# microsoft/crescent-credentials

Hardware: AMD Instinct MI355X
Metric: Groth16 proofs/sec (rs256-sd-shaped circuit, BN254), G1 MSM scalar-adds/sec reported alongside (higher is better)
Workload: dtype u32 limbs (BN254 Fq/Fr, 254-bit modular integers)

## Files before the change

crescent-credentials_amd/csrc/msm.hip:

```cpp
#include "msm.hpp"
#include "g2pair.hpp"

#include <chrono>
#include <cstring>
#include <type_traits>

namespace cg {

static constexpr int SCALAR_BITS = 255;

int msm_default_window(uint64_t n, bool precomputed) {
    double best = 1e300;
    int best_c = 4;
    for (int c = 4; c <= 22; ++c) {
        int W = (SCALAR_BITS + c - 1) / c;
        if ((double)W * (double)n >= 2147483648.0) continue;
        double buckets = (double)(1u << (c - 1)) * (precomputed ? 1 : W);
        if (buckets > (double)(1u << 24)) continue;
        double cost = (double)n * W * 12.0 + buckets * 2.0 * 16.0;
        if (cost < best) { best = cost; best_c = c; }
    }
    return best_c;
}

// ... 188 lines not shown
    if constexpr (I < N) {
        f(std::integral_constant<int, I>{});
        static_for<I + 1, N>(f);
    }
}
template <int C, class Fn>
__device__ __forceinline__ void for_each_digit_c(const uint32_t (&s)[8], Fn f) {
    constexpr int W = (SCALAR_BITS + C - 1) / C;
    constexpr uint32_t mask = (1u << C) - 1u, half = 1u << (C - 1);
    int hl = -1;
    uint32_t top = 0;
#pragma unroll
    for (int i = 0; i < 8; ++i) {
        hl = s[i] ? i : hl;
        top = s[i] ? s[i] : top;
    }
    if (hl < 0) return;
    const int topbit = hl * 32 + 31 - __clz((int)top);
    uint32_t carry = 0;
    bool live = true;
    static_for<0, W>([&](auto jc) __attribute__((always_inline)) {
        constexpr int j = decltype(jc)::value;
        constexpr int bit = C * j, lo = bit >> 5, sh = bit & 31;
        if (!live) return;
        if (bit > topbit && carry == 0) { live = false; return; }
        uint32_t w = 0;
        if constexpr (lo < 8) {
            if constexpr (sh == 0) w = s[lo];
            else if constexpr (lo + 1 < 8) w = __builtin_amdgcn_alignbit(s[lo + 1], s[lo], sh);
            else w = s[lo] >> sh;
        }
        const uint32_t raw = (w & mask) + carry;
        int32_t d;
        if (raw > half) { d = (int32_t)raw - (int32_t)(1u << C); carry = 1; }
        else { d = (int32_t)raw; carry = 0; }
        f(j, d);
    });
}

static constexpr int PART_MAX_BITS = 12;
static constexpr uint32_t PART_TILE = 4096;
static constexpr uint32_t PART_THREADS = 1024;
static constexpr uint32_t PART_CHUNK = 8192;
static constexpr uint32_t PART_PAD = 16;
enum { PLAN_N = 0, PLAN_L = 1, PLAN_T = 2, PLAN_NONZERO = 3, PLAN_CHUNKS = 4, PLAN_DONE = 5, PLAN_WORDS = 8 };

struct PartShape {
    uint32_t n;
    int c, W;
    int precomputed;
    uint32_t row_stride;
    int bits1, bits2;
    int staged;
};

__device__ __forceinline__ Fr load_scalar_or_zero(const Fr* __restrict__ scalars, uint32_t i, bool ok) {
    uint4 a = make_uint4(0u, 0u, 0u, 0u), b = a;
    if (ok) {
        const uint4* p = reinterpret_cast<const uint4*>(scalars + i);
        a = p[0];
        b = p[1];
    }
    Fr r;
    r.l[0] = a.x; r.l[1] = a.y; r.l[2] = a.z; r.l[3] = a.w;
    r.l[4] = b.x; r.l[5] = b.y; r.l[6] = b.z; r.l[7] = b.w;
    return r;
}

template <int C, class Fn>
__device__ __forceinline__ void for_each_entry(const PartShape& sh, const Fr& s, uint32_t i, Fn f) {
    const uint32_t nb = 1u << (sh.c - 1);
    auto emit = [&](int j, int32_t d) {
        if (d == 0) return;
        const uint32_t mag = (uint32_t)(d < 0 ? -d : d);
        const uint32_t sign = d < 0 ? 0x80000000u : 0u;
        if (sh.precomputed) f(mag - 1u, ((uint32_t)j * sh.row_stride + i) | sign);
        else f((uint32_t)j * nb + (mag - 1u), i | sign);
    };
    if constexpr (C > 0) for_each_digit_c<C>(s.l, emit);
    else for_each_digit(s.l, sh.c, sh.W, emit);
}

struct PlanArgs {
    uint32_t* start1;
    uint32_t* chunk0;
    uint32_t target_threads, min_L;
    int two_level;
};
__device__ __forceinline__ uint32_t block_exclusive_scan(uint32_t* sc, uint32_t n);
__device__ __forceinline__ void part_plan_block(int bits1, const PlanArgs& pa, const uint32_t* hist1, uint32_t* plan, uint32_t* lds);

template <int C>
__global__ void __launch_bounds__(PART_THREADS) k_part_count(PartShape sh, const Fr* __restrict__ scalars, const uint8_t* __restrict__ valid,
                                                    uint32_t* __restrict__ blk_hist, uint32_t* hist1, uint32_t* plan, PlanArgs pa) {
    extern __shared__ uint32_t lds[];
    const uint32_t B1 = 1u << sh.bits1;
    for (uint32_t k = threadIdx.x; k < B1; k += blockDim.x) lds[k] = 0;
    __syncthreads();
    const uint32_t base = blockIdx.x * PART_TILE;
    uint32_t nonzero = 0;
    constexpr int PER = PART_TILE / PART_THREADS;
    Fr sc[PER];
    bool ok[PER];
#pragma unroll
    for (int u = 0; u < PER; ++u) {
        const uint32_t i = base + u * PART_THREADS + threadIdx.x;
        ok[u] = i < sh.n && valid[i] != 0;
        sc[u] = load_scalar_or_zero(scalars, i, ok[u]);
    }
    static_for<0, PER>([&](auto uc) {
        constexpr int u = decltype(uc)::value;
        if (!ok[u]) return;
        bool any = false;
        for_each_entry<C>(sh, sc[u], base + u * PART_THREADS + threadIdx.x, [&](uint32_t key, uint32_t) {
            atomicAdd(&lds[key >> sh.bits2], 1u);
            any = true;
        });
        nonzero += any;
    });
    __shared__ uint32_t nz_block;
    if (threadIdx.x == 0) nz_block = 0;
    for (int off = 32; off > 0; off >>= 1) nonzero += __shfl_down((int)nonzero, off, 64);
    __syncthreads();
    if ((threadIdx.x & 63) == 0 && nonzero) atomicAdd(&nz_block, nonzero);
    __syncthreads();
    if (threadIdx.x == 0 && nz_block) atomicAdd(&plan[PLAN_NONZERO], nz_block);
    uint32_t* row = blk_hist + (size_t)blockIdx.x * B1;
    for (uint32_t k = threadIdx.x; k < B1; k += blockDim.x) {
        const uint32_t v = lds[k];
        row[k] = v;
        if (v) atomicAdd(&hist1[(size_t)k * PART_PAD], v);
    }
    __shared__ uint32_t is_last;
    __builtin_amdgcn_s_waitcnt(0x0F70);
    __builtin_amdgcn_fence(__ATOMIC_RELEASE, "workgroup");
    __syncthreads();
    if (threadIdx.x == 0)
        is_last = __hip_atomic_fetch_add(&plan[PLAN_DONE], 1u, __ATOMIC_RELAXED, __HIP_MEMORY_SCOPE_AGENT) == gridDim.x - 1u;
    __syncthreads();
    if (!is_last) return;
    part_plan_block(sh.bits1, pa, hist1, plan, lds);
}

__device__ __forceinline__ uint32_t block_exclusive_scan(uint32_t* sc, uint32_t n) {
    __shared__ uint32_t wave_tot[16];
    __shared__ uint32_t grand;
    const uint32_t per = (n + blockDim.x - 1) / blockDim.x;
    const uint32_t lo = threadIdx.x * per, hi = lo + per < n ? lo + per : n;
    uint32_t sum = 0;
    for (uint32_t k = lo; k < hi; ++k) sum += sc[k];
    uint32_t incl = sum;
    for (int off = 1; off < 64; off <<= 1) {
        uint32_t v = (uint32_t)__shfl_up((int)incl, off, 64);
        if ((threadIdx.x & 63) >= (uint32_t)off) incl += v;
    }
    if ((threadIdx.x & 63) == 63) wave_tot[threadIdx.x >> 6] = incl;
    __syncthreads();
    if (threadIdx.x == 0) {
        uint32_t run = 0;
        for (uint32_t w = 0; w < (blockDim.x + 63) / 64; ++w) { uint32_t t = wave_tot[w]; wave_tot[w] = run; run += t; }
        grand = run;
    }
    __syncthreads();
    uint32_t run = wave_tot[threadIdx.x >> 6] + incl - sum;
    for (uint32_t k = lo; k < hi; ++k) { uint32_t t = sc[k]; sc[k] = run; run += t; }
    __syncthreads();
    return grand;
}

__device__ __forceinline__ void part_plan_block(int bits1, const PlanArgs& pa, const uint32_t* hist1, uint32_t* plan, uint32_t* lds) {
    const uint32_t B1 = 1u << bits1;
    auto hist = [&](uint32_t k) { return __hip_atomic_load(&hist1[(size_t)k * PART_PAD], __ATOMIC_RELAXED, __HIP_MEMORY_SCOPE_AGENT); };
    __syncthreads();
    for (uint32_t k = threadIdx.x; k < B1; k += blockDim.x) lds[k] = hist(k);
    __syncthreads();
    const uint32_t N = block_exclusive_scan(lds, B1);
    for (uint32_t k = threadIdx.x; k < B1; k += blockDim.x) pa.start1[k] = lds[k];
    if (threadIdx.x == 0) {
        pa.start1[B1] = N;
        uint32_t L = (uint32_t)(((uint64_t)N + pa.target_threads - 1) / pa.target_threads);
        if (L < pa.min_L) L = pa.min_L;
        plan[PLAN_N] = N;
        plan[PLAN_L] = L;
        plan[PLAN_T] = N ? (N + L - 1) / L : 0;
    }
    if (!pa.two_level) return;
    __syncthreads();
    for (uint32_t k = threadIdx.x; k < B1; k += blockDim.x) lds[k] = (hist(k) + PART_CHUNK - 1) / PART_CHUNK;
    __syncthreads();
    const uint32_t chunks = block_exclusive_scan(lds, B1);
    for (uint32_t k = threadIdx.x; k < B1; k += blockDim.x) pa.chunk0[k] = lds[k];
    if (threadIdx.x == 0) { pa.chunk0[B1] = chunks; plan[PLAN_CHUNKS] = chunks; }
}

__global__ void k_replan(uint32_t* __restrict__ plan, const uint32_t* __restrict__ src_plan, uint32_t target_segments, uint32_t min_L) {
    for (int k = 0; k < PLAN_WORDS; ++k) plan[k] = src_plan[k];
    const uint32_t N = plan[PLAN_N];
    uint32_t L = (uint32_t)(((uint64_t)N + target_segments - 1) / target_segments);
    if (L < min_L) L = min_L;
    plan[PLAN_L] = L;
    plan[PLAN_T] = N ? (N + L - 1) / L : 0;
}

template <int C>
__global__ void __launch_bounds__(PART_THREADS) k_part_place(PartShape sh, const Fr* __restrict__ scalars, const uint8_t* __restrict__ valid,
                                                    const uint32_t* __restrict__ blk_hist, const uint32_t* __restrict__ start1,
                                                    uint32_t* __restrict__ cur1, uint64_t* __restrict__ out) {
    extern __shared__ uint32_t lds[];
    const uint32_t B1 = 1u << sh.bits1;
    const uint32_t* row = blk_hist + (size_t)blockIdx.x * B1;
    for (uint32_t k = threadIdx.x; k < B1; k += blockDim.x) {
        const uint32_t cnt = row[k];
        lds[k] = cnt ? start1[k] + atomicAdd(&cur1[(size_t)k * PART_PAD], cnt) : 0u;
    }
    const uint32_t base = blockIdx.x * PART_TILE;
    constexpr int PER = PART_TILE / PART_THREADS;
    Fr sc[PER];
    bool ok[PER];
#pragma unroll
    for (int u = 0; u < PER; ++u) {
        const uint32_t i = base + u * PART_THREADS + threadIdx.x;
        ok[u] = i < sh.n && valid[i] != 0;
        sc[u] = load_scalar_or_zero(scalars, i, ok[u]);
    }
    __syncthreads();
    static_for<0, PER>([&](auto uc) {
        constexpr int u = decltype(uc)::value;
        if (!ok[u]) return;
        for_each_entry<C>(sh, sc[u], base + u * PART_THREADS + threadIdx.x, [&](uint32_t key, uint32_t val) {
            const uint32_t pos = atomicAdd(&lds[key >> sh.bits2], 1u);
            out[pos] = ((uint64_t)key << 32) | val;
        });
    });
}

static constexpr uint32_t STAGE_SUB = 1024;
static constexpr int STAGE_MIN_C = 18;
template <int C>
__global__ void __launch_bounds__(PART_THREADS) k_part_place_staged(PartShape sh, const Fr* __restrict__ scalars, const uint8_t* __restrict__ valid,
                                                           const uint32_t* __restrict__ blk_hist, const uint32_t* __restrict__ start1,
                                                           uint32_t* __restrict__ cur1, uint64_t* __restrict__ out) {
    constexpr int W = (SCALAR_BITS + C - 1) / C;
    extern __shared__ __attribute__((aligned(16))) uint32_t lds[];
    const uint32_t B1 = 1u << sh.bits1;
    uint32_t* gbase = lds;
    uint32_t* cnt = lds + B1;
    uint32_t* off = lds + 2 * B1;
    uint64_t* stage = reinterpret_cast<uint64_t*>(lds + 3 * B1 + (B1 & 1u));
    const uint32_t* row = blk_hist + (size_t)blockIdx.x * B1;
    for (uint32_t k = threadIdx.x; k < B1; k += blockDim.x) {
        const uint32_t c = row[k];
        gbase[k] = c ? start1[k] + atomicAdd(&cur1[(size_t)k * PART_PAD], c) : 0u;
    }
    const uint32_t base = blockIdx.x * PART_TILE;
    for (uint32_t sub = 0; sub < PART_TILE / STAGE_SUB; ++sub) {
        const uint32_t i = base + sub * STAGE_SUB + threadIdx.x;
        for (uint32_t k = threadIdx.x; k < B1; k += blockDim.x) cnt[k] = 0;
        __syncthreads();
        uint64_t e[W];
#pragma unroll
        for (int u = 0; u < W; ++u) e[u] = ~0ull;
        if (i < sh.n && valid[i] != 0) {
            const Fr sc = scalars[i];
            for_each_digit_c<C>(sc.l, [&](int j, int32_t d) {
                if (d == 0) return;
                const uint32_t key = (uint32_t)(d < 0 ? -d : d) - 1u;
                const uint32_t val = ((uint32_t)j * sh.row_stride + i) | (d < 0 ? 0x80000000u : 0u);
                e[j] = ((uint64_t)key << 32) | val;
                atomicAdd(&cnt[key >> sh.bits2], 1u);
            });
        }
        __syncthreads();
        for (uint32_t k = threadIdx.x; k < B1; k += blockDim.x) off[k] = cnt[k];
        __syncthreads();
        const uint32_t total = block_exclusive_scan(off, B1);
        for (uint32_t k = threadIdx.x; k < B1; k += blockDim.x) cnt[k] = off[k];
        __syncthreads();
#pragma unroll
        for (int u = 0; u < W; ++u)
            if (e[u] != ~0ull) stage[atomicAdd(&cnt[(uint32_t)(e[u] >> 32) >> sh.bits2], 1u)] = e[u];
        __syncthreads();
        for (uint32_t k = threadIdx.x; k < total; k += blockDim.x) {
            const uint64_t v = stage[k];
            const uint32_t b = (uint32_t)(v >> 32) >> sh.bits2;
            out[gbase[b] + (k - off[b])] = v;
        }
// ... 796 lines not shown
    for (int k = 0; k < PLAN_WORDS; ++k) h_plan.p[k] = 0;
    h_result.alloc((size_t)wins * (red_rbits + red_cbits1) * ACC);
    if (!ev_t[0])
        for (auto& e : ev_t) CG_HIP(hipEventCreate(&e));
}

template <class F>
void MsmEngine<F>::device_bytes(uint64_t& entries, uint64_t& pieces, uint64_t& other) const {
    entries += own_mem.entry_bytes();
    pieces += own_mem.piece_bytes();
    other += blk_hist.bytes() + counters.bytes() + starts.bytes() + bucket_sums.bytes() + rows_buf.bytes() + cols_buf.bytes() +
             rowp_buf.bytes() + colp_buf.bytes();
}

static float elapsed_ms(hipEvent_t a, hipEvent_t b) {
    float ms = 0;
    if (hipEventElapsedTime(&ms, a, b) != hipSuccess) return 0.f;
    return ms;
}
template <class F> float MsmEngine<F>::ms_total() const { return elapsed_ms(ev_t[0], ev_t[5]); }
template <class F> float MsmEngine<F>::ms_sort() const { return n_scalars ? elapsed_ms(ev_t[1], ev_t[2]) : 0.f; }
template <class F> float MsmEngine<F>::ms_accum() const { return n_scalars ? elapsed_ms(ev_t[3], ev_t[4]) : 0.f; }

template <class F>
MsmEngine<F>::~MsmEngine() {
    for (auto& e : ev_t) if (e) (void)hipEventDestroy(e);
}

template <class F>
void MsmEngine<F>::digits(const Fr* scalars_dev, uint64_t n, hipStream_t st) {
    if (n > bases->n) n = bases->n;
    n_scalars = n;
    adopted = nullptr;
    for (int k = 0; k < PLAN_WORDS; ++k) h_plan.p[k] = 0;
    CG_HIP(hipEventRecord(ev_t[0], st));
    if (!n) {
        if (!counters_clean) fill_zero(counters.p, (counters.bytes() + 15) & ~(size_t)15, st);
        counters_clean = zero_at_end;
        return;
    }
    const uint32_t B1 = 1u << bits1;
    uint32_t* plan = counters.p;
    uint32_t* hist1 = plan + PLAN_WORDS;
    uint32_t* cur1 = hist1 + (size_t)B1 * PART_PAD;
    uint32_t* hist2 = cur1 + (size_t)B1 * PART_PAD;
    uint32_t* cur2 = hist2 + (bits2 ? ((size_t)1 << (bits1 + bits2)) : 0);
    uint32_t* start1 = starts.p;
    uint32_t* chunk0 = starts.p + B1 + 1;
    PartShape sh;
    sh.n = (uint32_t)n; sh.c = bases->c; sh.W = bases->W; sh.precomputed = bases->precomputed ? 1 : 0;
    sh.row_stride = (uint32_t)bases->n;
    sh.bits1 = bits1; sh.bits2 = bits2;
    sh.staged = latency_mode ? 1 : 0;
    const uint32_t tiles = ceil_div(n, PART_TILE);
    CG_HIP(hipEventRecord(ev_t[1], st));
    if (!counters_clean) fill_zero(counters.p, (counters.bytes() + 15) & ~(size_t)15, st);
    counters_clean = false;
    PlanArgs pa;
    pa.start1 = start1; pa.chunk0 = chunk0; pa.target_threads = acc_target_segments<F29T>(latency_mode); pa.min_L = min_L;
    pa.two_level = bits2 ? 1 : 0;
    launch_part_level1(true, sh, tiles, (size_t)B1 * 4, st, scalars_dev, bases->valid.p, blk_hist.p, hist1, plan, nullptr, nullptr, nullptr, pa);
    CG_KERNEL_CHECK();
    launch_part_level1(false, sh, tiles, (size_t)B1 * 4, st, scalars_dev, bases->valid.p, blk_hist.p, nullptr, nullptr, start1, cur1, mem().ent_a.p, pa);
    CG_KERNEL_CHECK();
    if (bits2) {
        const uint32_t B2 = 1u << bits2;
        k_part_count2<<<max_chunks, 256, (size_t)B2 * 4, st>>>(bits1, bits2, mem().ent_a.p, chunk0, start1, hist2);
        CG_KERNEL_CHECK();
        k_part_place2<<<max_chunks, 256, (size_t)B2 * 16 + (size_t)PART_CHUNK * 8, st>>>(bits1, bits2, mem().ent_a.p, chunk0, start1, hist2, cur2, mem().ent_b.p);
        CG_KERNEL_CHECK();
    }
    CG_HIP(hipEventRecord(ev_t[2], st));
}

template <class F>
void MsmEngine<F>::adopt(const uint64_t* grouped_entries, const uint32_t* plan_dev, uint64_t n, hipStream_t st) {
    if (n > bases->n) n = bases->n;
    n_scalars = n;
    for (int k = 0; k < PLAN_WORDS; ++k) h_plan.p[k] = 0;
    CG_HIP(hipEventRecord(ev_t[0], st));
    CG_HIP(hipEventRecord(ev_t[1], st));
    k_replan<<<1, 1, 0, st>>>(counters.p, plan_dev, acc_target_segments<F29T>(latency_mode), min_L);
    counters_clean = false;
    CG_KERNEL_CHECK();
    CG_HIP(hipEventRecord(ev_t[2], st));
    adopted = n ? grouped_entries : nullptr;
}

static bool red_force_tree() {
    static const bool v = CG_TUNE_ENV("RED_TREE") != nullptr;
    return v;
}

template <class F>
void MsmEngine<F>::accumulate(hipStream_t st, bool defer_reduction) {
    reduction_pending = false;
    if (!buckets_clean) fill_zero(bucket_sums.p, bucket_sums.bytes(), st);
    buckets_clean = false;
    if (n_scalars) {
        const uint32_t* plan = counters.p;
        const uint64_t* grouped = adopted ? adopted : this->grouped();
        CG_HIP(hipEventRecord(ev_t[3], st));
        static const bool knock_accum = CG_TUNE_ENV("KNOCK_ACCUM") != nullptr, knock_combine = CG_TUNE_ENV("KNOCK_COMBINE") != nullptr;
        if (!knock_accum)
            launch_accum_affine<F29T>(grouped, plan, max_segments, bases->table.p, bucket_sums.p, mem().part_keys_a.p, mem().part_pts_a.p, latency_mode, st);
        CG_KERNEL_CHECK();
// ... 285 lines not shown
```

crescent-credentials_amd/csrc/msm.hpp:

```cpp
#pragma once
#include "common.hpp"
#include "curve29.hpp"
#include "ntt.hpp"

#include <functional>

namespace cg {

template <class F>
struct MsmBases {
    typedef typename To29<F>::type F29T;
    static constexpr int AFF = Words29<F29T>::AFF;
    uint64_t n = 0;
    int c = 0;
    int W = 0;
    bool precomputed = true;
    DevBuf<uint32_t> table;
    DevBuf<uint8_t> valid;
    void build(const Affine<F>* bases_dev, uint64_t n, int c, bool precompute, hipStream_t st);
    void build_from_row0(const uint32_t* row0_dev, const uint8_t* valid_dev, uint64_t n, int c, hipStream_t st);
    int rebuild(int c_new, hipStream_t st);
    void alloc_rows(uint64_t n, int c, bool precompute);
    void expand_rows(hipStream_t st);
};

int msm_default_window(uint64_t n, bool precomputed);
int msm_best_window(uint64_t n_bases, double nz_small, double nz_full);

struct MsmScratch {
    DevBuf<uint64_t> ent_a, ent_b;
    DevBuf<uint32_t> part_keys_a, part_keys_b;
    DevBuf<uint32_t> part_pts_a, part_pts_b;
    uint64_t entry_bytes() const { return ent_a.bytes() + ent_b.bytes(); }
    uint64_t piece_bytes() const { return part_keys_a.bytes() + part_keys_b.bytes() + part_pts_a.bytes() + part_pts_b.bytes(); }
    void reserve(size_t n_ent_a, size_t n_ent_b, size_t keys_a, size_t pts_a, size_t keys_b, size_t pts_b) {
        if (ent_a.n < n_ent_a) ent_a.alloc(n_ent_a);
        if (ent_b.n < n_ent_b) ent_b.alloc(n_ent_b);
        if (part_keys_a.n < keys_a) part_keys_a.alloc(keys_a);
        if (part_pts_a.n < pts_a) part_pts_a.alloc(pts_a);
        if (part_keys_b.n < keys_b) part_keys_b.alloc(keys_b);
        if (part_pts_b.n < pts_b) part_pts_b.alloc(pts_b);
    }
};

template <class F>
struct MsmEngine {
    typedef typename To29<F>::type F29T;
    static constexpr int ACC = Words29<F29T>::ACC;
    const MsmBases<F>* bases = nullptr;
    uint64_t cap_entries = 0;
    uint32_t nbuckets_total = 0;
    MsmScratch own_mem;
    MsmScratch* shared_mem = nullptr;
    MsmScratch& mem() { return shared_mem ? *shared_mem : own_mem; }
    const MsmScratch& mem() const { return shared_mem ? *shared_mem : own_mem; }
    int bits1 = 0, bits2 = 0;
    DevBuf<uint32_t> blk_hist;
    DevBuf<uint32_t> counters;
    DevBuf<uint32_t> starts;
    uint32_t max_chunks = 0;
    uint32_t min_L = 16;
    uint32_t max_segments = 0;
    DevBuf<uint32_t> bucket_sums;
    DevBuf<uint32_t> rows_buf, cols_buf;
    DevBuf<uint32_t> rowp_buf, colp_buf;
    int red_rbits = 0, red_cbits1 = 0;
    PinnedBuf<uint32_t> h_plan;
    PinnedBuf<uint32_t> h_result;
    uint64_t n_scalars = 0;
    bool zero_at_end = false;
    bool counters_clean = false, buckets_clean = false;
    bool latency_mode = false;
    uint32_t n_entries() const { return h_plan.p ? h_plan.p[0] : 0; }
    uint32_t n_nonzero() const { return h_plan.p ? h_plan.p[3] : 0; }
    void enqueue_reduction(hipStream_t st);
    bool reduction_pending = false;
    hipEvent_t ev_t[6] = {nullptr, nullptr, nullptr, nullptr, nullptr, nullptr};
    float ms_total() const;
    float ms_sort() const;
    float ms_accum() const;

    void init(const MsmBases<F>* b, hipStream_t zero_stream = nullptr);
    ~MsmEngine();
    void device_bytes(uint64_t& entries, uint64_t& pieces, uint64_t& other) const;
    void digits(const Fr* scalars_dev, uint64_t n, hipStream_t st);
    template <class G>
    bool can_adopt(const MsmEngine<G>& src) const {
        return bases->precomputed && src.bases->precomputed && bases->n == src.bases->n && bases->c == src.bases->c &&
               bits1 == src.bits1 && bits2 == src.bits2;
    }
    void adopt(const uint64_t* grouped_entries, const uint32_t* plan_dev, uint64_t n, hipStream_t st);
    const uint64_t* grouped() const { return bits2 ? mem().ent_b.p : mem().ent_a.p; }
    const uint64_t* adopted = nullptr;
    void accumulate(hipStream_t st, bool defer_reduction = false);
    XYZZ<F> value() const;
};

void enqueue_reduction_batch(MsmEngine<Fq>* const* engines, int n, hipStream_t st);

void ec_inverse_dft(const uint32_t* row0_in, const uint8_t* valid_in, uint64_t n_in, int logn, const Fr& scale_base,
                    const Fr& scale_mult, uint32_t* row0_out, uint8_t* valid_out, hipStream_t st);
void ec_transform_h_bases(const uint32_t* row0_in, const uint8_t* valid_in, uint64_t n_in, int logn, uint32_t* row0_out,
                          uint8_t* valid_out, hipStream_t st);
void ec_fold_c_into_l(const uint32_t* h_row0, const uint8_t* h_valid, uint64_t n_h, int logn, const Fr& vanishing_inv,
                      const cg_csr& c_matrix, uint64_t num_constraints, uint64_t num_inputs, uint64_t M,
                      const uint32_t* l_row0, const uint8_t* l_valid, uint32_t* row0_out, uint8_t* valid_out, hipStream_t st);
void ec_fold_ct_into_l(const uint32_t* h_row0, const uint8_t* h_valid, uint64_t n_h, int logn, const Fr& vanishing_inv,
                       const HostCsc& c_transposed, uint64_t num_constraints, uint64_t num_inputs, uint64_t M,
                       const uint32_t* l_row0, const uint8_t* l_valid, uint32_t* row0_out, uint8_t* valid_out, hipStream_t st);
void sum_xyzz_by_key(const uint32_t* keys, const uint32_t* pts, uint64_t count, uint32_t* sums, hipStream_t st);
void build_hl_bases_folded(MsmBases<Fq>& out_h, MsmBases<Fq>& out_l, const Affine<Fq>* h_bases_dev, uint64_t n_h, int logn,
                           const Affine<Fq>* l_bases_dev, uint64_t num_inputs, uint64_t M, const cg_csr& c_matrix,
                           uint64_t num_constraints, const Fr& vanishing_inv, uint64_t h_first, uint64_t h_stride, uint64_t h_count,
                           int c_h, uint64_t l_first, uint64_t l_count, int c_l, hipStream_t st, float* ms_fold = nullptr,
                           float* ms_tables = nullptr);

void build_h_bases_folded(MsmBases<Fq>& out_h, const uint32_t* h_row0, const uint8_t* h_valid, uint64_t n_h, int logn, uint64_t h_first,
                          uint64_t h_stride, uint64_t h_count, int c_h, hipStream_t st, float* ms_fold, float* ms_tables);
void build_l_bases_folded(MsmBases<Fq>& out_l, const uint32_t* h_row0, const uint8_t* h_valid, uint64_t n_h, int logn,
                          const uint32_t* l_row0, const uint8_t* l_valid, uint64_t num_inputs, uint64_t M, const HostCsc& c_transposed,
                          uint64_t num_constraints, const Fr& vanishing_inv, uint64_t l_first, uint64_t l_count,
                          const std::function<int()>& pick_c_l, hipStream_t st, float* ms_fold, float* ms_tables);

template <class F>
void import_bases(const uint8_t* host_bytes, uint32_t coord_form, uint64_t n, Affine<F>* out_dev, hipStream_t st);
// ... 8 lines not shown
```

crescent-credentials_amd/csrc/prover.hip:

```cpp
#include <atomic>
#include <condition_variable>
#include <shared_mutex>
#include <memory>
#include <mutex>
#include <chrono>
#include <cstdlib>
#include <exception>
#include <functional>
#include <thread>

#include "msm.hpp"
#include "ntt.hpp"
#include "scalar_form.hpp"
#include "wmap29.hpp"

namespace cg {

const char* csr_view_problem(const cg_csr& m);

std::string& last_error() {
    static thread_local std::string e;
    return e;
}
int fail(int code, const char* fmt, ...) {
// ... 357 lines not shown

template <class F>
static void load_query(MsmBases<F>& bases, const uint8_t* bytes, uint32_t form, uint64_t first, uint64_t count, int window_bits,
                       bool precompute, hipStream_t st, float* ms_copy, float* ms_tables) {
    constexpr size_t PT = sizeof(Affine<F>);
    auto t0 = std::chrono::steady_clock::now();
    DevBuf<Affine<F>> tmp(count ? count : 1);
    import_bases<F>(bytes + first * PT, form, count, tmp.p, st);
    if (ms_copy) *ms_copy += ms_since(t0);
    t0 = std::chrono::steady_clock::now();
    int c = window_bits > 0 ? window_bits : msm_default_window(count ? count : 1, precompute);
    bases.build(tmp.p, count, c, precompute, st);
    CG_HIP(hipStreamSynchronize(st));
    if (ms_tables) *ms_tables += ms_since(t0);
}

struct SlotRecipe { size_t dev_bytes = 0, host_bytes = 0; };
static std::unique_ptr<ProofSlot> make_slot(cg_ctx* c, const KeyTables& tables, hipStream_t zs, SlotRecipe& rec, bool lone = false,
                                            const std::vector<hipStream_t>& borrow = {}) {
    CG_HIP(hipSetDevice(c->device));
    std::unique_ptr<ProofSlot> sl(new ProofSlot());
    sl->lone = lone;
    AllocMeter meter;
    if (rec.dev_bytes) {
        sl->arena.reset(new SlotArena());
        DevBuf<uint8_t> whole(rec.dev_bytes);
        sl->arena->dev = whole.p; sl->arena->dev_size = rec.dev_bytes;
        whole.p = nullptr; whole.n = 0;
        if (rec.host_bytes) {
            CG_HIP(hipHostMalloc((void**)&sl->arena->host, rec.host_bytes, hipHostMallocDefault));
            sl->arena->host_size = rec.host_bytes;
        }
    }
    ArenaScope carve(sl->arena.get(), rec.dev_bytes ? nullptr : &meter);
    bool serial = !c->latency && !lone;
    if (const char* e = CG_TUNE_ENV("SERIAL_STREAMS")) serial = e[0] == '1' && !lone;
    const bool chain_prio = CG_TUNE_ENV("CHAIN_PRIORITY") && CG_TUNE_ENV("CHAIN_PRIORITY")[0] == '1';
    int prio_lo = 0, prio_hi = 0;
    (void)hipDeviceGetStreamPriorityRange(&prio_lo, &prio_hi);
    for (int i = 0; i < 5; ++i) {
        if (serial && i) sl->st[i] = sl->st[0];
        else if ((size_t)i < borrow.size()) { sl->st[i] = borrow[i]; sl->st_borrowed[i] = true; }
        else if (chain_prio && i == 0) CG_HIP(hipStreamCreateWithPriority(&sl->st[i], hipStreamNonBlocking, prio_hi));
        else CG_HIP(hipStreamCreateWithFlags(&sl->st[i], hipStreamNonBlocking));
    }
    CG_HIP(hipEventCreateWithFlags(&sl->ev_w, hipEventDisableTiming));
    CG_HIP(hipEventCreateWithFlags(&sl->ev_b1, hipEventDisableTiming));
    CG_HIP(hipEventCreateWithFlags(&sl->ev_done, hipEventDisableTiming));
    for (auto& e : sl->ev_fin) CG_HIP(hipEventCreateWithFlags(&e, hipEventDisableTiming));
    sl->one_stream = serial;
    for (auto& e : sl->ev_t) CG_HIP(hipEventCreate(&e));
    const bool latency = c->latency || lone;
    const bool zero_at_end = serial && !(CG_TUNE_ENV("NO_ZERO_AT_END") && CG_TUNE_ENV("NO_ZERO_AT_END")[0] == '1');
    each_query([&](int, auto& e, const auto& t) {
        e.latency_mode = latency;
        if (serial) e.shared_mem = &sl->scratch;
        e.zero_at_end = zero_at_end;
        e.init(&t, zs);
    }, *sl, tables);
    if (c->external_q) {
        sl->h_canon.alloc(c->rh.hi - c->rh.lo ? c->rh.hi - c->rh.lo : 1);
        sl->wm.h_bad_input.alloc(1);
    } else {
        sl->h_canon.alloc(c->D);
        sl->wm.alloc(c->M, c->D, std::max(c->A.sell_scratch, std::max(c->B.sell_scratch, c->C.sell_scratch)));
    }
    if (!rec.dev_bytes) { rec.dev_bytes = meter.dev_bytes + 4096; rec.host_bytes = meter.host_bytes + 4096; }
    return sl;
}

static void add_lone_slot(cg_ctx* c, std::vector<std::unique_ptr<ProofSlot>>& slots, const KeyTables& tables, hipStream_t zs) {
    if (c->n_lone <= 0) return;
    try {
        SlotRecipe own;
        size_t next = slots.size();
        for (int k = 0; k < c->n_lone; ++k) {
            std::vector<hipStream_t> borrow;
            while (borrow.size() < 5 && next > 2 && !slots[next - 1]->lone) borrow.push_back(slots[--next]->st[0]);
            slots.push_back(make_slot(c, tables, zs, own, true, borrow));
        }
    } catch (const HipError& e) {
        if (e.code != CG_ERR_OUT_OF_MEMORY) throw;
        (void)hipGetLastError();
    }
}

struct JoinAll {
    std::vector<std::thread> th;
    ~JoinAll() { for (auto& t : th) if (t.joinable()) t.join(); }
};

struct WorkerCancelled {};
static void staged_worker(cg_ctx* c) {
    const auto t0 = std::chrono::steady_clock::now();
    int status = 0;
    std::string err;
    bool done = false, from_proof = false;
    float ms_fold = 0.f, ms_tables = 0.f, ms_slots = 0.f, ms_wait = 0.f;
    try {
        CG_HIP(hipSetDevice(c->device));
        KeyTables tables;
        const KeyTables& row0 = c->tables;
        std::vector<std::unique_ptr<ProofSlot>> slots;
        int64_t table_bytes = 0;
        auto stop = [&] { if (c->cancel.load()) throw WorkerCancelled(); };
        const uint64_t D = c->D, M = c->M, l = c->l;
        const int wb = c->window_opt;
        TuneStats ts;
// ... 1111 lines not shown
```

crescent-credentials_amd/csrc/wmap29.hip:

```cpp
#include "wmap29.hpp"
#include "satcheck.hpp"

namespace cg {

static constexpr int TS29_SMALL = 10, TS29_BIG = 11;
static int strided_max_stages(int tile_log) { return tile_log == TS29_BIG ? 10 : 6; }
static int ntt_passes(int logn, int tile_log) {
    if (logn <= tile_log) return 1;
    const int smax = strided_max_stages(tile_log);
    return 1 + (logn - tile_log + smax - 1) / smax;
}
static int ntt_tile_log(int logn) {
    static const int forced = [] {
        const char* e = CG_TUNE_ENV("NTT_TILE");
        return (e && (atoi(e) == TS29_SMALL || atoi(e) == TS29_BIG)) ? atoi(e) : 0;
    }();
    if (forced) return (forced == TS29_BIG && logn > TS29_SMALL) ? TS29_BIG : TS29_SMALL;
    return (logn >= 20 && ntt_passes(logn, TS29_BIG) < ntt_passes(logn, TS29_SMALL)) ? TS29_BIG : TS29_SMALL;
}

__device__ __forceinline__ Fr29 load_packed29(const uint32_t* __restrict__ base, uint64_t idx) {
    const uint4* p = reinterpret_cast<const uint4*>(base + idx * 8);
    uint4 a = p[0], b = p[1];
    uint32_t w[8] = {a.x, a.y, a.z, a.w, b.x, b.y, b.z, b.w};
// ... 58 lines not shown
        k_to_packed29<<<ceil_div(n, 256), 256, 0, st>>>(d.icoset_br.p, icoset.p, n, 1, logn);
    }
    CG_KERNEL_CHECK();
    Fr29 v = from_mont256<Fr29P>(d.vanishing_inv);
    pack29(v, vinv);
    Fr vp = from_mont(d.vanishing_inv);
    memcpy(vinv_plain, vp.l, 32);
}

void Wm29Strided::build(const NttDomain& big, int logs_, int rank, hipStream_t st) {
    logs = logs_;
    d = big.n >> logs;
    NttDomain small;
    small.build(big.logn - logs, false, st);
    sub.build(small, st);
    const Fr s = mul(fr_from_u64(5), fr_pow_u64(fr_root_of_unity(big.logn), (uint64_t)rank));
    DevBuf<Fr> t(big.n);
    fr_pow_table(t.p, s, inv(fr_from_u64(big.n)), big.n, false, big.logn, st);
    fold.alloc(big.n * 8);
    k_to_packed29<<<ceil_div(big.n, 256), 256, 0, st>>>(t.p, fold.p, big.n, 0, 0);
    CG_KERNEL_CHECK();
    CG_HIP(hipStreamSynchronize(st));
}

__global__ void __launch_bounds__(256) k_fold29(const uint32_t* __restrict__ a, const uint32_t* __restrict__ T, uint32_t* __restrict__ out,
                                                uint32_t d, int logd, uint32_t terms) {
    const uint32_t i = blockIdx.x * blockDim.x + threadIdx.x;
    if (i >= d) return;
    Fr29 acc = Fr29::zero();
    for (uint32_t t = 0; t < terms; ++t) {
        const uint64_t e = (uint64_t)i + (uint64_t)t * d;
        acc = add(acc, mul(load_packed29(a, e), load_packed29(T, e)));
        if ((t & 3u) == 3u) acc = normalize(acc);
        if ((t & 63u) == 63u) acc = weak_reduce(acc);
    }
    store_packed29(out, brev(i, logd), weak_reduce(normalize(acc)));
}

void Csr29::build(const DevCsr& m, hipStream_t st) {
    dict.alloc(m.dict.n * 8);
    k_to_packed29<<<ceil_div(m.dict.n, 256), 256, 0, st>>>(m.dict.p, dict.p, m.dict.n, 0, 0);
    CG_KERNEL_CHECK();
}

__device__ __forceinline__ bool fr_lt_modulus(const Fr& x) {
    bool lt = false, decided = false;
#pragma unroll
    for (int k = 7; k >= 0; --k) {
        if (!decided && x.l[k] != FrP::N[k]) { lt = x.l[k] < FrP::N[k]; decided = true; }
    }
    return lt;
}

__global__ void __launch_bounds__(256) k_w_to29(const Fr* __restrict__ w, uint32_t* __restrict__ out, uint64_t n,
                                                uint32_t* __restrict__ bad_input, uint32_t* __restrict__ va, uint64_t m, uint64_t l, int logn) {
    uint64_t i = (uint64_t)blockIdx.x * blockDim.x + threadIdx.x;
    if (i >= n) return;
    Fr x = w[i];
    if (!fr_lt_modulus(x)) *bad_input = 1u;
    const Fr29 v = mul(unpack29<Fr29P>(x.l), Fr29::from_limbs(Fr29P::R2));
    store_packed29(out, i, v);
    if (i < l) store_packed29(va, brev((uint32_t)(m + i), logn), v);
}


__global__ void __launch_bounds__(256) k_sell29(const uint32_t* __restrict__ slice_ptr, const uint32_t* __restrict__ col,
                                                const uint32_t* __restrict__ cidx, const uint32_t* __restrict__ dst,
                                                const uint32_t* __restrict__ dict, const uint32_t* __restrict__ src,
                                                uint32_t* __restrict__ out, uint32_t* __restrict__ scratch, uint32_t n_pieces, int logn) {
    const uint32_t p = blockIdx.x * blockDim.x + threadIdx.x;
    if (p >= n_pieces) return;
    const uint32_t s = p >> 6, lane = p & 63u;
    const uint32_t base = slice_ptr[s], len = (slice_ptr[s + 1] - base) >> 6;
    Fr29 acc = Fr29::zero();
    uint32_t cnt = 0;
#if !defined(CG_SELL_BATCH)
#define CG_SELL_BATCH 0
#endif
#if CG_SELL_BATCH == 0
    for (uint32_t t = 0; t < len; ++t) {
        const uint32_t ci = cidx[base + t * 64 + lane];
        if (ci == SELL_PAD) continue;
        Fr29 v = load_packed29(src, col[base + t * 64 + lane]);
        if (ci != 0) v = mul(v, load_packed29(dict, ci));
        acc = add(acc, v);
        if ((++cnt & 3u) == 0) acc = normalize(acc);
    }
#else
    constexpr uint32_t BS = CG_SELL_BATCH;
    uint32_t ci[SELL_PIECE], cl[SELL_PIECE];
#pragma unroll
    for (uint32_t t = 0; t < SELL_PIECE; ++t) {
        const bool in = t < len;
        ci[t] = in ? cidx[base + t * 64 + lane] : SELL_PAD;
        cl[t] = in ? col[base + t * 64 + lane] : 0u;
    }
#pragma unroll
    for (uint32_t h = 0; h < SELL_PIECE; h += BS) {
        if (h >= len) break;
        uint4 rv[BS][2], rd[BS][2];
#pragma unroll
        for (uint32_t u = 0; u < BS; ++u) {
            const uint32_t t = h + u;
            if (ci[t] == SELL_PAD) continue;
            const uint4* pv = reinterpret_cast<const uint4*>(src + (uint64_t)cl[t] * 8);
            rv[u][0] = pv[0]; rv[u][1] = pv[1];
            if (ci[t] != 0) {
                const uint4* pd = reinterpret_cast<const uint4*>(dict + (uint64_t)ci[t] * 8);
                rd[u][0] = pd[0]; rd[u][1] = pd[1];
            }
        }
#pragma unroll
        for (uint32_t u = 0; u < BS; ++u) {
            const uint32_t t = h + u;
            if (ci[t] == SELL_PAD) continue;
// ... 210 lines not shown
    if (threadIdx.x == 0) { rec[0] = 0ull; rec[1] = ~0ull; }
}
__global__ void __launch_bounds__(256) k_sat_check29(const uint32_t* __restrict__ va, const uint32_t* __restrict__ vb,
                                                     const uint32_t* __restrict__ vc, uint64_t D, uint64_t m, int logn,
                                                     unsigned long long* __restrict__ rec) {
    const uint64_t j = (uint64_t)blockIdx.x * blockDim.x + threadIdx.x;
    const uint32_t i = j < D ? brev((uint32_t)j, logn) : 0xffffffffu;
    bool bad = false;
    if (j < D && (uint64_t)i < m) {
        const uint4* pa = reinterpret_cast<const uint4*>(va + j * 8);
        const uint4* pb = reinterpret_cast<const uint4*>(vb + j * 8);
        const uint4* pc = reinterpret_cast<const uint4*>(vc + j * 8);
        const uint4 a0 = pa[0], a1 = pa[1], b0 = pb[0], b1 = pb[1], c0 = pc[0], c1 = pc[1];
        const uint32_t a[8] = {a0.x, a0.y, a0.z, a0.w, a1.x, a1.y, a1.z, a1.w};
        const uint32_t b[8] = {b0.x, b0.y, b0.z, b0.w, b1.x, b1.y, b1.z, b1.w};
        const uint32_t c[8] = {c0.x, c0.y, c0.z, c0.w, c1.x, c1.y, c1.z, c1.w};
        bad = !sat_row_ok(a, b, c);
    }
    const unsigned long long failing = __ballot(bad);
    if (failing == 0ull) return;
    uint32_t first = bad ? i : 0xffffffffu;
#pragma unroll
    for (int off = 32; off > 0; off >>= 1) first = min(first, (uint32_t)__shfl_xor((int)first, off, 64));
    if ((threadIdx.x & 63u) == 0u) {
        atomicAdd(&rec[0], (unsigned long long)__popcll(failing));
        atomicMin(&rec[1], (unsigned long long)first);
    }
}
__global__ void k_sat_row29(const uint32_t* __restrict__ va, const uint32_t* __restrict__ vb, const uint32_t* __restrict__ vc,
                            const unsigned long long* __restrict__ rec, uint64_t m, int logn, uint32_t* __restrict__ out) {
    if (threadIdx.x != 0 || blockIdx.x != 0) return;
    if (rec[0] == 0ull || rec[1] >= m) {
        for (int k = 0; k < 24; ++k) out[k] = 0u;
        return;
    }
    const uint64_t j = brev((uint32_t)rec[1], logn);
    const uint32_t* v[3] = {va, vb, vc};
    for (int k = 0; k < 3; ++k) {
        uint32_t in[8], o[8];
        for (int t = 0; t < 8; ++t) in[t] = v[k][j * 8 + t];
        sat_row_value(in, o);
        for (int t = 0; t < 8; ++t) out[k * 8 + t] = o[t];
    }
}

static void wm29_products(const Wm29Domain& dom, const DevCsr& A, const DevCsr& B, const DevCsr& C, const Csr29& dA, const Csr29& dB,
                          const Csr29& dC, Wm29Buffers& buf, const Fr* w_canon, uint64_t M, uint64_t m, uint64_t l, hipStream_t st, int nvec,
                          int half) {
    const uint64_t D = dom.n;
    const int logn = dom.logn;
    buf.h_bad_input.p[0] = 0;
    uint32_t* v[3] = {buf.va.p, buf.vb.p, buf.vc.p};
    fill_zero(v[0], D * 32, st);
    k_w_to29<<<ceil_div(M, 256), 256, 0, st>>>(w_canon, buf.w29.p, M, buf.h_bad_input.dev(), buf.va.p, m, l, logn);
    CG_KERNEL_CHECK();
    const DevCsr* mats[3] = {&A, &B, &C};
    const Csr29* dicts[3] = {&dA, &dB, &dC};
    for (int k = 0; k < nvec; ++k) {
        if (half && k != half - 1) continue;
        if (k) fill_zero(v[k], D * 32, st);
        const uint32_t* src = buf.w29.p;
        for (int lv = 0; lv < mats[k]->n_sell; ++lv) {
            const SellLevel& L = mats[k]->sell[lv];
            uint32_t* scratch = (lv & 1) ? buf.sp_b.p : buf.sp_a.p;
            if (L.n_partials > buf.sp_cap) throw HipError(CG_ERR_INVALID_ARGUMENT, "sparse-product scratch smaller than the matrix needs");
            if (L.n_pieces) {
                k_sell29<<<ceil_div(L.n_pieces, 256), 256, 0, st>>>(L.slice_ptr.p, L.col.p, L.cidx.p, L.dst.p, dicts[k]->dict.p, src, v[k],
                                                                    scratch, L.n_pieces, logn);
                CG_KERNEL_CHECK();
            }
            src = scratch;
        }
    }
}
static void wm29_queue_check(const Wm29Domain& dom, Wm29Buffers& buf, uint64_t m, hipStream_t st) {
    k_sat_init29<<<1, 64, 0, st>>>(buf.sat.rec.p);
    k_sat_check29<<<ceil_div(dom.n, 256), 256, 0, st>>>(buf.va.p, buf.vb.p, buf.vc.p, dom.n, m, dom.logn, buf.sat.rec.p);
    CG_KERNEL_CHECK();
    CG_HIP(hipMemcpyAsync(buf.sat.h_rec.p, buf.sat.rec.p, 2 * sizeof(unsigned long long), hipMemcpyDeviceToHost, st));
}

void wm29_check(const Wm29Domain& dom, const DevCsr& A, const DevCsr& B, const DevCsr& C, const Csr29& dA, const Csr29& dB, const Csr29& dC,
                Wm29Buffers& buf, const Fr* w_canon, uint64_t M, uint64_t m, uint64_t l, hipStream_t st) {
    wm29_products(dom, A, B, C, dA, dB, dC, buf, w_canon, M, m, l, st, 3, 0);
    wm29_queue_check(dom, buf, m, st);
    k_sat_row29<<<1, 64, 0, st>>>(buf.va.p, buf.vb.p, buf.vc.p, buf.sat.rec.p, m, dom.logn, buf.sat.row.p);
    CG_KERNEL_CHECK();
    CG_HIP(hipMemcpyAsync(buf.sat.h_row.p, buf.sat.row.p, 24 * sizeof(uint32_t), hipMemcpyDeviceToHost, st));
}

void wm29_run(const Wm29Domain& dom, const DevCsr& A, const DevCsr& B, const DevCsr& C, const Csr29& dA, const Csr29& dB,
              const Csr29& dC, Wm29Buffers& buf, const Fr* w_canon, uint64_t M, uint64_t m, uint64_t l, Fr* h_out,
              hipStream_t st, bool coset_values, const Wm29Strided* strided, int half, bool check_witness) {
    uint32_t* v[3] = {buf.va.p, buf.vb.p, buf.vc.p};
    if (check_witness && half) throw HipError(CG_ERR_INVALID_ARGUMENT, "one half of the witness map cannot check the witness");
    const int nvec = (coset_values && !check_witness) ? 2 : 3;
    wm29_products(dom, A, B, C, dA, dB, dC, buf, w_canon, M, m, l, st, nvec, half);
    if (check_witness) wm29_queue_check(dom, buf, m, st);
    if (coset_values && strided) {
        const Wm29Strided& S = *strided;
        const uint32_t d = (uint32_t)S.d;
        const int logd = S.sub.logn;
        const uint32_t terms = 1u << S.logs;
        dit29(dom, dom.tw_inv.p, buf.va.p, nullptr, nullptr, false, buf.va.p, buf.vt.p, nullptr, false, st);
        k_fold29<<<ceil_div(d, 256), 256, 0, st>>>(buf.vt.p, S.fold.p, buf.va.p, d, logd, terms);
        CG_KERNEL_CHECK();
        dit29(S.sub, S.sub.tw_fwd.p, buf.va.p, nullptr, nullptr, false, buf.va.p, buf.vc.p, nullptr, false, st, dom.vinv_plain);
// ... 90 lines not shown
```

Baseline: 180.5.

## Compact wide-digit scalars in MSM partition and witness Montgomery conversion

MSM partition count/place kernels now classify each scalar as zero, single-small-digit, or wide. Small scalars (typical of circuit witnesses, mostly 0/1 or bits) get a single direct bucket update, and wide scalars are compacted into an LDS list so that their digit walk runs without lane divergence. The witness-to-Montgomery conversion likewise writes zeros directly, computes the Montgomery form of one once per block, and only multiplies the remaining values. This adds ballot/atomic/LDS overhead and extra syncs. It is disabled for the dense H query and can be switched off with an environment variable.

```diff
diff --git a/crescent-credentials_amd/csrc/msm.hip b/crescent-credentials_amd/csrc/msm.hip
--- a/crescent-credentials_amd/csrc/msm.hip
+++ b/crescent-credentials_amd/csrc/msm.hip
@@ -264,7 +264,37 @@
     uint32_t row_stride;
     int bits1, bits2;
     int staged;
+    int compact;
 };
+
+static constexpr uint32_t PART_COMPACT_MAX = PART_TILE / 2;
+enum { DIGITS_NONE = 0, DIGITS_NARROW = 1, DIGITS_WIDE = 2 };
+template <int C>
+__device__ __forceinline__ int digit_class(const Fr& s, bool ok) {
+    const uint32_t hi = s.l[1] | s.l[2] | s.l[3] | s.l[4] | s.l[5] | s.l[6] | s.l[7];
+    if (!ok || (hi | s.l[0]) == 0) return DIGITS_NONE;
+    return (hi == 0 && s.l[0] <= (1u << (C - 1))) ? DIGITS_NARROW : DIGITS_WIDE;
+}
+template <int PER>
+__device__ __forceinline__ void append_wide(const int (&cls)[PER], uint16_t* list, uint32_t* n_wide) {
+    uint64_t m[PER];
+    uint32_t tot = 0;
+#pragma unroll
+    for (int u = 0; u < PER; ++u) {
+        m[u] = __ballot(cls[u] == DIGITS_WIDE);
+        tot += (uint32_t)__popcll(m[u]);
+    }
+    if (tot == 0) return;
+    const uint32_t lane = threadIdx.x & 63u;
+    uint32_t at = 0;
+    if (lane == 0) at = atomicAdd(n_wide, tot);
+    at = (uint32_t)__shfl((int)at, 0, 64);
+#pragma unroll
+    for (int u = 0; u < PER; ++u) {
+        if (cls[u] == DIGITS_WIDE) list[at + (uint32_t)__popcll(m[u] & ((1ull << lane) - 1ull))] = (uint16_t)(u * PART_THREADS + threadIdx.x);
+        at += (uint32_t)__popcll(m[u]);
+    }
+}
 
 __device__ __forceinline__ Fr load_scalar_or_zero(const Fr* __restrict__ scalars, uint32_t i, bool ok) {
     uint4 a = make_uint4(0u, 0u, 0u, 0u), b = a;
@@ -277,6 +307,23 @@
     r.l[0] = a.x; r.l[1] = a.y; r.l[2] = a.z; r.l[3] = a.w;
     r.l[4] = b.x; r.l[5] = b.y; r.l[6] = b.z; r.l[7] = b.w;
     return r;
+}
+
+template <int PER>
+__device__ __forceinline__ void load_tile(const PartShape& sh, const Fr* __restrict__ scalars, const uint8_t* __restrict__ valid,
+                                          uint32_t base, Fr (&sc)[PER], bool (&ok)[PER]) {
+    uint32_t at[PER];
+    uint8_t flag[PER];
+#pragma unroll
+    for (int u = 0; u < PER; ++u) {
+        const uint32_t i = base + u * PART_THREADS + threadIdx.x;
+        at[u] = i < sh.n ? i : sh.n - 1u;
+        flag[u] = valid[at[u]];
+    }
+#pragma unroll
+    for (int u = 0; u < PER; ++u) sc[u] = load_scalar_or_zero(scalars, at[u], true);
+#pragma unroll
+    for (int u = 0; u < PER; ++u) ok[u] = base + u * PART_THREADS + threadIdx.x < sh.n && flag[u] != 0;
 }
 
 template <int C, class Fn>
@@ -306,30 +353,59 @@
 __global__ void __launch_bounds__(PART_THREADS) k_part_count(PartShape sh, const Fr* __restrict__ scalars, const uint8_t* __restrict__ valid,
                                                     uint32_t* __restrict__ blk_hist, uint32_t* hist1, uint32_t* plan, PlanArgs pa) {
     extern __shared__ uint32_t lds[];
+    __shared__ uint16_t wide_list[C > 0 ? PART_TILE : 1];
+    __shared__ uint32_t n_wide;
     const uint32_t B1 = 1u << sh.bits1;
     for (uint32_t k = threadIdx.x; k < B1; k += blockDim.x) lds[k] = 0;
+    if constexpr (C > 0)
+        if (threadIdx.x == 0) n_wide = 0;
     __syncthreads();
     const uint32_t base = blockIdx.x * PART_TILE;
     uint32_t nonzero = 0;
     constexpr int PER = PART_TILE / PART_THREADS;
     Fr sc[PER];
     bool ok[PER];
-#pragma unroll
-    for (int u = 0; u < PER; ++u) {
-        const uint32_t i = base + u * PART_THREADS + threadIdx.x;
-        ok[u] = i < sh.n && valid[i] != 0;
-        sc[u] = load_scalar_or_zero(scalars, i, ok[u]);
-    }
-    static_for<0, PER>([&](auto uc) {
-        constexpr int u = decltype(uc)::value;
-        if (!ok[u]) return;
+    load_tile<PER>(sh, scalars, valid, base, sc, ok);
+    auto count_walk = [&](const Fr& s, uint32_t i) {
         bool any = false;
-        for_each_entry<C>(sh, sc[u], base + u * PART_THREADS + threadIdx.x, [&](uint32_t key, uint32_t) {
+        for_each_entry<C>(sh, s, i, [&](uint32_t key, uint32_t) {
             atomicAdd(&lds[key >> sh.bits2], 1u);
             any = true;
         });
         nonzero += any;
-    });
+    };
+    auto walk_in_place = [&]() {
+        static_for<0, PER>([&](auto uc) {
+            constexpr int u = decltype(uc)::value;
+            if (ok[u]) count_walk(sc[u], base + u * PART_THREADS + threadIdx.x);
+        });
+    };
+    bool compact = false;
+    if constexpr (C > 0) compact = sh.compact != 0;
+    if (!compact) {
+        walk_in_place();
+    } else {
+        int cls[PER];
+#pragma unroll
+        for (int u = 0; u < PER; ++u) cls[u] = digit_class<C ? C : 1>(sc[u], ok[u]);
+        append_wide<PER>(cls, wide_list, &n_wide);
+        __syncthreads();
+        const uint32_t nw = n_wide;
+        if (nw > PART_COMPACT_MAX) {
+            walk_in_place();
+        } else {
+#pragma unroll
+            for (int u = 0; u < PER; ++u)
+                if (cls[u] == DIGITS_NARROW) {
+                    atomicAdd(&lds[(sc[u].l[0] - 1u) >> sh.bits2], 1u);
+                    ++nonzero;
+                }
+            for (uint32_t k = threadIdx.x; k < nw; k += blockDim.x) {
+                const uint32_t i = base + wide_list[k];
+                count_walk(load_scalar_or_zero(scalars, i, true), i);
+            }
+        }
+    }
     __shared__ uint32_t nz_block;
     if (threadIdx.x == 0) nz_block = 0;
     for (int off = 32; off > 0; off >>= 1) nonzero += __shfl_down((int)nonzero, off, 64);
@@ -419,6 +495,13 @@
                                                     const uint32_t* __restrict__ blk_hist, const uint32_t* __restrict__ start1,
                                                     uint32_t* __restrict__ cur1, uint64_t* __restrict__ out) {
     extern __shared__ uint32_t lds[];
+    __shared__ uint16_t wide_list[C > 0 ? PART_TILE : 1];
+    __shared__ uint32_t n_wide;
+    const bool compact = C > 0 && sh.compact;
+    if (compact) {
+        if (threadIdx.x == 0) n_wide = 0;
+        __syncthreads();
+    }
     const uint32_t B1 = 1u << sh.bits1;
     const uint32_t* row = blk_hist + (size_t)blockIdx.x * B1;
     for (uint32_t k = threadIdx.x; k < B1; k += blockDim.x) {
@@ -429,21 +512,39 @@
     constexpr int PER = PART_TILE / PART_THREADS;
     Fr sc[PER];
     bool ok[PER];
-#pragma unroll
-    for (int u = 0; u < PER; ++u) {
-        const uint32_t i = base + u * PART_THREADS + threadIdx.x;
-        ok[u] = i < sh.n && valid[i] != 0;
-        sc[u] = load_scalar_or_zero(scalars, i, ok[u]);
-    }
-    __syncthreads();
-    static_for<0, PER>([&](auto uc) {
-        constexpr int u = decltype(uc)::value;
-        if (!ok[u]) return;
-        for_each_entry<C>(sh, sc[u], base + u * PART_THREADS + threadIdx.x, [&](uint32_t key, uint32_t val) {
-            const uint32_t pos = atomicAdd(&lds[key >> sh.bits2], 1u);
-            out[pos] = ((uint64_t)key << 32) | val;
+    load_tile<PER>(sh, scalars, valid, base, sc, ok);
+    auto place = [&](uint32_t key, uint32_t val) {
+        const uint32_t pos = atomicAdd(&lds[key >> sh.bits2], 1u);
+        out[pos] = ((uint64_t)key << 32) | val;
+    };
+    auto walk_in_place = [&]() {
+        static_for<0, PER>([&](auto uc) {
+            constexpr int u = decltype(uc)::value;
+            if (ok[u]) for_each_entry<C>(sh, sc[u], base + u * PART_THREADS + threadIdx.x, place);
         });
-    });
+    };
+    if (!compact) {
+        __syncthreads();
+        walk_in_place();
+    } else {
+        int cls[PER];
+#pragma unroll
+        for (int u = 0; u < PER; ++u) cls[u] = digit_class<C ? C : 1>(sc[u], ok[u]);
+        append_wide<PER>(cls, wide_list, &n_wide);
+        __syncthreads();
+        const uint32_t nw = n_wide;
+        if (nw > PART_COMPACT_MAX) {
+            walk_in_place();
+        } else {
+#pragma unroll
+            for (int u = 0; u < PER; ++u)
+                if (cls[u] == DIGITS_NARROW) place(sc[u].l[0] - 1u, base + u * PART_THREADS + threadIdx.x);
+            for (uint32_t k = threadIdx.x; k < nw; k += blockDim.x) {
+                const uint32_t i = base + wide_list[k];
+                for_each_entry<C>(sh, load_scalar_or_zero(scalars, i, true), i, place);
+            }
+        }
+    }
 }
 
 static constexpr uint32_t STAGE_SUB = 1024;
@@ -1346,6 +1447,8 @@
     sh.row_stride = (uint32_t)bases->n;
     sh.bits1 = bits1; sh.bits2 = bits2;
     sh.staged = latency_mode ? 1 : 0;
+    static const bool no_compaction = CG_TUNE_ENV("NO_DIGIT_COMPACTION") && CG_TUNE_ENV("NO_DIGIT_COMPACTION")[0] == '1';
+    sh.compact = (dense_scalars || no_compaction) ? 0 : 1;
     const uint32_t tiles = ceil_div(n, PART_TILE);
     CG_HIP(hipEventRecord(ev_t[1], st));
     if (!counters_clean) fill_zero(counters.p, (counters.bytes() + 15) & ~(size_t)15, st);
diff --git a/crescent-credentials_amd/csrc/msm.hpp b/crescent-credentials_amd/csrc/msm.hpp
--- a/crescent-credentials_amd/csrc/msm.hpp
+++ b/crescent-credentials_amd/csrc/msm.hpp
@@ -71,6 +71,7 @@
     bool zero_at_end = false;
     bool counters_clean = false, buckets_clean = false;
     bool latency_mode = false;
+    bool dense_scalars = false;
     uint32_t n_entries() const { return h_plan.p ? h_plan.p[0] : 0; }
     uint32_t n_nonzero() const { return h_plan.p ? h_plan.p[3] : 0; }
     void enqueue_reduction(hipStream_t st);
diff --git a/crescent-credentials_amd/csrc/prover.hip b/crescent-credentials_amd/csrc/prover.hip
--- a/crescent-credentials_amd/csrc/prover.hip
+++ b/crescent-credentials_amd/csrc/prover.hip
@@ -433,8 +433,9 @@
     for (auto& e : sl->ev_t) CG_HIP(hipEventCreate(&e));
     const bool latency = c->latency || lone;
     const bool zero_at_end = serial && !(CG_TUNE_ENV("NO_ZERO_AT_END") && CG_TUNE_ENV("NO_ZERO_AT_END")[0] == '1');
-    each_query([&](int, auto& e, const auto& t) {
+    each_query([&](int q, auto& e, const auto& t) {
         e.latency_mode = latency;
+        e.dense_scalars = q == Q_H;
         if (serial) e.shared_mem = &sl->scratch;
         e.zero_at_end = zero_at_end;
         e.init(&t, zs);
diff --git a/crescent-credentials_amd/csrc/wmap29.hip b/crescent-credentials_amd/csrc/wmap29.hip
--- a/crescent-credentials_amd/csrc/wmap29.hip
+++ b/crescent-credentials_amd/csrc/wmap29.hip
@@ -134,15 +134,78 @@
     return lt;
 }
 
+__device__ __forceinline__ void store_words29(uint32_t* __restrict__ base, uint64_t idx, const uint4& lo, const uint4& hi) {
+    uint4* p = reinterpret_cast<uint4*>(base + idx * 8);
+    p[0] = lo;
+    p[1] = hi;
+}
 __global__ void __launch_bounds__(256) k_w_to29(const Fr* __restrict__ w, uint32_t* __restrict__ out, uint64_t n,
-                                                uint32_t* __restrict__ bad_input, uint32_t* __restrict__ va, uint64_t m, uint64_t l, int logn) {
-    uint64_t i = (uint64_t)blockIdx.x * blockDim.x + threadIdx.x;
-    if (i >= n) return;
-    Fr x = w[i];
-    if (!fr_lt_modulus(x)) *bad_input = 1u;
-    const Fr29 v = mul(unpack29<Fr29P>(x.l), Fr29::from_limbs(Fr29P::R2));
-    store_packed29(out, i, v);
-    if (i < l) store_packed29(va, brev((uint32_t)(m + i), logn), v);
+                                                uint32_t* __restrict__ bad_input, uint32_t* __restrict__ va, uint64_t m, uint64_t l, int logn,
+                                                int compact) {
+    const uint64_t base = (uint64_t)blockIdx.x * blockDim.x;
+    const uint64_t i = base + threadIdx.x;
+    if (!compact) {
+        if (i >= n) return;
+        Fr x = w[i];
+        if (!fr_lt_modulus(x)) *bad_input = 1u;
+        const Fr29 v = mul(unpack29<Fr29P>(x.l), Fr29::from_limbs(Fr29P::R2));
+        store_packed29(out, i, v);
+        if (i < l) store_packed29(va, brev((uint32_t)(m + i), logn), v);
+        return;
+    }
+    __shared__ uint8_t list[256];
+    __shared__ uint32_t n_list;
+    __shared__ uint4 one29[2];
+    if (threadIdx.x == 0) n_list = 0;
+    __syncthreads();
+    bool is_one = false, other = false;
+    if (i < n) {
+        const Fr x = w[i];
+        if (!fr_lt_modulus(x)) *bad_input = 1u;
+        const uint32_t hi = x.l[1] | x.l[2] | x.l[3] | x.l[4] | x.l[5] | x.l[6] | x.l[7];
+        is_one = hi == 0 && x.l[0] == 1u;
+        other = hi != 0 || x.l[0] > 1u;
+        if (!is_one && !other) {
+            const uint4 z = make_uint4(0u, 0u, 0u, 0u);
+            store_words29(out, i, z, z);
+            if (i < l) store_words29(va, brev((uint32_t)(m + i), logn), z, z);
+        }
+    }
+    const uint64_t mask = __ballot(other);
+    if (mask) {
+        const uint32_t lane = threadIdx.x & 63u;
+        uint32_t at = 0;
+        if (lane == 0) at = atomicAdd(&n_list, (uint32_t)__popcll(mask));
+        at = (uint32_t)__shfl((int)at, 0, 64);
+        if (other) list[at + (uint32_t)__popcll(mask & ((1ull << lane) - 1ull))] = (uint8_t)threadIdx.x;
+    }
+    __syncthreads();
+    const uint32_t nl = n_list;
+    for (uint32_t k = threadIdx.x; k <= nl; k += blockDim.x) {
+        const uint64_t j = k < nl ? base + list[k] : base;
+        Fr x = w[j];
+        if (k == nl) {
+#pragma unroll
+            for (int t = 0; t < 8; ++t) x.l[t] = t == 0 ? 1u : 0u;
+        }
+        const Fr29 v = mul(unpack29<Fr29P>(x.l), Fr29::from_limbs(Fr29P::R2));
+        uint32_t p[8];
+        pack29(v, p);
+        const uint4 lo = make_uint4(p[0], p[1], p[2], p[3]), hi = make_uint4(p[4], p[5], p[6], p[7]);
+        if (k < nl) {
+            store_words29(out, j, lo, hi);
+            if (j < l) store_words29(va, brev((uint32_t)(m + j), logn), lo, hi);
+        } else {
+            one29[0] = lo;
+            one29[1] = hi;
+        }
+    }
+    __syncthreads();
+    if (is_one) {
+        const uint4 lo = one29[0], hi = one29[1];
+        store_words29(out, i, lo, hi);
+        if (i < l) store_words29(va, brev((uint32_t)(m + i), logn), lo, hi);
+    }
 }
 
 
@@ -459,7 +522,8 @@
     buf.h_bad_input.p[0] = 0;
     uint32_t* v[3] = {buf.va.p, buf.vb.p, buf.vc.p};
     fill_zero(v[0], D * 32, st);
-    k_w_to29<<<ceil_div(M, 256), 256, 0, st>>>(w_canon, buf.w29.p, M, buf.h_bad_input.dev(), buf.va.p, m, l, logn);
+    static const bool no_compaction = CG_TUNE_ENV("NO_DIGIT_COMPACTION") && CG_TUNE_ENV("NO_DIGIT_COMPACTION")[0] == '1';
+    k_w_to29<<<ceil_div(M, 256), 256, 0, st>>>(w_canon, buf.w29.p, M, buf.h_bad_input.dev(), buf.va.p, m, l, logn, no_compaction ? 0 : 1);
     CG_KERNEL_CHECK();
     const DevCsr* mats[3] = {&A, &B, &C};
     const Csr29* dicts[3] = {&dA, &dB, &dC};
```

Result: faster. 185.5, median of 6 (+2.8%).
